# GreenleafLab/NucleoATAC

Measured on AMD Instinct MI355X. Metric: Mbp/s through occ+nuc signal pipeline, higher is better.
Workload: dtype f64

## Files before the change

nucleoatac_amd/csrc/natac_api.hip:

```cpp
#include "../../include/natac.h"
#ifndef NATAC_GNBL
#define NATAC_GNBL 2
#endif
#include "natac_kernels.hpp"
#include "natac_fft_bg.hpp"
#include "natac_occ_fast.hpp"
#include "natac_cand.hpp"
#include "natac_covsweep.hpp"
#include "natac_textz.hpp"
#include "natac_cores.hpp"
#include "natac_writer.hpp"
#include "natac_tabix.hpp"
#include "natac_pack.hpp"
#include "natac_bam.hpp"
#include "natac_bam_dev.hpp"
#include "natac_fasta.hpp"
#include "natac_fuzzfit.hpp"
#include "natac_bedtab.hpp"
#include "natac_pwmfit.hpp"
#include "natac_sites.hpp"
#include "natac_tracks.hpp"

#include <algorithm>
#include <cmath>
#include <cstdarg>
#include <cstdio>
#include <cstring>
#include <limits>
#include <string>
#include <vector>

using namespace natac;

static thread_local std::string g_err;

static int fail(int code, const char *fmt, ...) {
    char buf[512];
    va_list ap;
    va_start(ap, fmt);
    vsnprintf(buf, sizeof buf, fmt, ap);
    va_end(ap);
    g_err = buf;
    return code;
}

#define HIPCHK(expr)                                                                                  \
    do {                                                                                              \
        hipError_t e_ = (expr);                                                                       \
        if (e_ != hipSuccess)                                                                         \
            return fail(e_ == hipErrorOutOfMemory ? NATAC_E_NOMEM : NATAC_E_HIP, "%s: %s (%s:%d)", #expr, \
                        hipGetErrorString(e_), __FILE__, __LINE__);                                   \
    } while (0)

static hipError_t pool_alloc(void **p, size_t bytes);
static void dev_free(void *p);

template <class T>
class PoolBuf {
  public:
    PoolBuf() = default;
    PoolBuf(PoolBuf &&o) noexcept : p_(o.p_), n_(o.n_) { o.p_ = nullptr; o.n_ = 0; }
    PoolBuf &operator=(PoolBuf &&o) noexcept {
        if (this != &o) { reset(); p_ = o.p_; n_ = o.n_; o.p_ = nullptr; o.n_ = 0; }
        return *this;
    }
    ~PoolBuf() { reset(); }
    void reset() { dev_free(p_); p_ = nullptr; n_ = 0; }
    hipError_t alloc(size_t n) {
        reset();
        if (n == 0) n = 1;
        void *p = nullptr;
        const hipError_t e = pool_alloc(&p, n * sizeof(T));
        if (e == hipSuccess) { p_ = (T *)p; n_ = n; }
        return e;
    }
    T *get() const { return p_; }
    operator T *() const { return p_; }
    size_t size() const { return n_; }

  private:
    T *p_ = nullptr;
    size_t n_ = 0;
};

template <class T>
static int dev_alloc(PoolBuf<T> &buf, size_t n) {
    HIPCHK(buf.alloc(n));
    return NATAC_OK;
}

struct natac_ctx {
    int device = 0;
    hipStream_t stream = nullptr;
    hipStream_t copy_stream = nullptr;
    hipDeviceProp_t prop;
    PoolBuf<double> d_vmat, d_vmat_pad, d_srow, d_sizes;
    PoolBuf<double> d_lrt;
    long long lrt_gen = -1;
    int vlower = 0, vupper = 0, vw = 0, R = 0, W = 0, sizes_upper = 0;
    bool have_vmat = false, have_sizes = false, srow_dirty = true;
    bool vmat_zero = false, srow_zero = false;
    long long model_gen = 0;
    PoolBuf<double> d_fft_tw, d_fft_k;
    PoolBuf<double> d_fft_mtab, d_fft_swt;
    bool bg_ext = true;
    bool fft_dirty = true, bg_direct = false, occ_ordered = true, occ_zero_nfr = false;
    std::vector<double> h_sizes;
    PoolBuf<double> d_nucp, d_nfrp, d_alphas;
    int occ_upper = 0, n_alpha = 0, step = 0, halfstep = 0, flank = 0;
    double cutoff = 0;
    bool have_occ = false;
    int occ_zero_flags = 0;
    PoolBuf<double> d_occ_q4, d_occ_rho;
    int occ_nm = 0;
    bool occ_fast_ok = false, occ_force_general = false, occ_rn16 = false;
    double occ_b_floor = 0;
    PoolBuf<double> d_win_nuc, d_win_occ;
    PoolBuf<double> d_wb_occ;
    int wb_M = 0, wb_step = 0;
    int win_nuc_M = 0, win_occ_M = 0;
    double win_nuc_sd = -1, win_occ_sd = -1;
    double win_nuc_sum = 0, win_occ_sum = 0;
    bool profiling = false;
    struct Ev { int k; hipEvent_t a, b; hipStream_t st; };
    std::vector<Ev> pending;
    double prof_ms[NATAC_K_COUNT] = {0};
    int64_t prof_n[NATAC_K_COUNT] = {0};
    hipEvent_t t0 = nullptr, t1 = nullptr;
    hipStream_t ck_stream = nullptr;
    hipEvent_t ck_start = nullptr;
    long long *d_ck = nullptr;
    int ck_cap = 0;
    bool ck_active = false;
    struct Iv { int k; float t0, t1; };
    std::vector<Iv> ck_iv;
    PoolBuf<natac_text::P10> d_p10;
    PoolBuf<natac_deflate::CrcTables> d_crc;
};

struct natac_bam {
    natac_bamio::Bam *impl = nullptr;
};

enum TrackState : unsigned char { TS_EMPTY = 0, TS_PENDING, TS_RUN , TS_HOST  };
struct BatchOutputs {
    TrackState track[NATAC_T_COUNT] = {};
    bool grids = false;
    long long bg_gen = -1;
    int nuc_w = -1, nuc_upper = -1;
    bool occ_cov_by_nuc = false;
};

struct natac_batch {
    natac_ctx *ctx = nullptr;
    int nc = 0;
    long long nf = 0, nb = 0, total_bp = 0, total_grid = 0;
    int bias_left = 0, bias_right = 0;
    std::vector<int> h_len;
    std::vector<long long> h_out_off, h_grid_off;
    PoolBuf<int> d_len, d_lpos, d_ilen, d_centre, d_status;
    PoolBuf<long long> d_frag_off, d_bias_off, d_out_off, d_grid_off;
    PoolBuf<double> d_bias, d_ebias;
    PoolBuf<unsigned long long> d_occ_minkey;
    PoolBuf<int> d_occ_nan;
    int n_tiles_os = 0, os_width = 0;
    PoolBuf<int2> d_tiles_os, d_tiles1k;
    int n_tiles1k = 0;
    PoolBuf<int2> d_tiles256, d_tiles_bg, d_tiles_occ, d_ranges_occ, d_ranges256;
    PoolBuf<long long> d_tile256_first;
    PoolBuf<int> d_order_occ;
    int ranges256_w = -1;
    int ranges_occ_key[3] = {-1, -1, -1};
    int n_tiles256 = 0, n_tiles_bg = 0, n_tiles_occ = 0, bgG = 0;
    int grid_step = 0, grid_half = 0;
    PoolBuf<long long> d_blk_off;
    long long total_blocks = 0;
    PoolBuf<double> d_gsum;
    PoolBuf<int2> d_tiles_gs;
    int n_tiles_gs = 0, gs_Q = -1;
    PoolBuf<int> d_defer;
// ... 102 lines not shown
}

static hipError_t pool_mem_info(int dev, size_t *avail, size_t *total) {
    size_t fr = 0, tot = 0;
    hipError_t e = hipMemGetInfo(&fr, &tot);
    if (e != hipSuccess) return e;
    std::lock_guard<std::mutex> lk(g_pool.mu);
    for (auto &kv : g_pool.free_blocks[dev & 15]) fr += kv.first;
    *avail = fr;
    *total = tot;
    return hipSuccess;
}

static void dev_free(void *p) {
    if (!p) return;
    std::lock_guard<std::mutex> lk(g_pool.mu);
    auto it = g_pool.live.find(p);
    if (it == g_pool.live.end()) { (void)hipFree(p); return; }
    const int dev = it->second.first;
    const size_t bytes = it->second.second;
    g_pool.live.erase(it);
    if (g_pool.enabled) g_pool.free_blocks[dev].insert({bytes, p});
    else (void)hipFree(p);
}

template <class T>
static int dev_upload(natac_ctx *c, PoolBuf<T> &buf, const T *src, size_t n) {
    int rc = dev_alloc(buf, n);
    if (rc) return rc;
    if (n) HIPCHK(hipMemcpyAsync(buf, src, n * sizeof(T), hipMemcpyHostToDevice, c->stream));
    return NATAC_OK;
}

class StreamTemps {
  public:
    explicit StreamTemps(natac_ctx *c) : c_(c) {}
    ~StreamTemps() {
        if (!bufs_.empty() && hipStreamQuery(c_->stream) != hipSuccess) (void)hipStreamSynchronize(c_->stream);
    }
    template <class T>
    int alloc(T **p, size_t n) {
        bufs_.emplace_back();
        int rc = dev_alloc(bufs_.back(), std::max<size_t>(n, 1) * sizeof(T));
        *p = (T *)bufs_.back().get();
        return rc;
    }
    template <class T>
    int upload(T **p, const T *src, size_t n) {
        int rc = alloc(p, n);
        if (rc) return rc;
        if (n) HIPCHK(hipMemcpyAsync(*p, src, n * sizeof(T), hipMemcpyHostToDevice, c_->stream));
        return NATAC_OK;
    }

  private:
    natac_ctx *c_;
    std::vector<PoolBuf<unsigned char>> bufs_;
};

static int choose_bg_G(const natac_batch *b, int W) {
    const int cand[4] = {7, 9, 13, 17};
    double best = 1e300;
    int bestG = 9;
    const int stride = std::max(1, b->nc / 65536);
    for (int ci = 0; ci < 4; ++ci) {
        const int G = cand[ci], TW = 64 * G;
        double cost = 0;
        for (int i = 0; i < b->nc; i += stride) {
            const int nt = (b->h_len[i] + TW - 1) / TW;
            cost += (double)nt * (TW + (W - 1) * 0.15 * 8);
        }
        if (cost < best) { best = cost; bestG = G; }
    }
    return bestG;
}

static void launch_candidates(natac_ctx *c, const ChunkTable &ct, const VMatDev &vm, const int *d_cc, const int *d_cp, long long n,
                              const double *nuc_cov, const double *norm, const double *bnum, const double *bcov, double *lr,
                              double *var, double *z, const long long *tile_first = nullptr, const int2 *ranges256 = nullptr) {
    const int EW = c->W + ((c->vupper - 2) >> 1) + ((c->vupper - 1) >> 1);
    const int ZN = (((c->vupper - 2) >> 1) + ((c->vupper - 1) >> 1) + 5 + 32) & ~1, ON = (c->W + 1) & ~1;
    const size_t lds4 = ((size_t)4 * CAND_PER_WAVE * ((EW + 1) & ~1) + ZN + ON) * sizeof(double);
    const bool per_wave = c->W <= 2 * WAVE;
    const size_t ldsp = (size_t)4 * CAND_PER_WAVE * CANDP_STRIDE * sizeof(double);
    bool paired = per_wave && bnum && bcov && c->vlower >= 2 && (c->R & 1) == 0 && c->W >= 64 && !vm.has_zero && EW <= CANDP_STRIDE &&
                  !getenv("NATAC_CAND_FULL") && !getenv("NATAC_CAND_OLD");
    if (paired && (c->lrt_gen != c->model_gen || !c->d_lrt)) {
        if (c->d_lrt.size() < (size_t)c->R * c->W && dev_alloc(c->d_lrt, (size_t)c->R * c->W) != NATAC_OK)
            paired = false;
        if (paired) {
            hipLaunchKernelGGL(natac_lr_table, dim3((unsigned)((c->R * c->W + 255) / 256)), dim3(256), 0, c->stream, c->d_vmat, c->d_srow, c->R, c->W,
                               c->d_lrt);
            c->lrt_gen = c->model_gen;
        }
    }
    if (paired) {
        VMatDev vml = vm;
        vml.lrt = c->d_lrt;
        const long long per_block = 4 * CAND_PER_WAVE;
        const dim3 grid((unsigned)((n + per_block - 1) / per_block));
        if (c->vlower & 1)
            hipLaunchKernelGGL((natac_candidates_paired<true>), grid, dim3(256), ldsp, c->stream, ct, vml, d_cc, d_cp, (int)n, nuc_cov, norm,
                               bnum, bcov, tile_first, ranges256, lr, var, z);
        else
            hipLaunchKernelGGL((natac_candidates_paired<false>), grid, dim3(256), ldsp, c->stream, ct, vml, d_cc, d_cp, (int)n, nuc_cov, norm,
                               bnum, bcov, tile_first, ranges256, lr, var, z);
        return;
    }
    if (per_wave && lds4 <= 64 * 1024) {
        const long long per_block = 4 * CAND_PER_WAVE;
        if (bnum && bcov && !getenv("NATAC_CAND_FULL"))
            hipLaunchKernelGGL((natac_candidates4<true>), dim3((unsigned)((n + per_block - 1) / per_block)), dim3(256), lds4, c->stream,
                               ct, vm, d_cc, d_cp, (int)n, nuc_cov, norm, bnum, bcov, lr, var, z);
        else
            hipLaunchKernelGGL((natac_candidates4<false>), dim3((unsigned)((n + per_block - 1) / per_block)), dim3(256), lds4, c->stream,
                               ct, vm, d_cc, d_cp, (int)n, nuc_cov, norm, bnum, bcov, lr, var, z);
    } else {
        hipLaunchKernelGGL(natac_candidates, dim3((unsigned)n), dim3(256), (size_t)(EW + 2) * sizeof(double), c->stream, ct, vm, d_cc,
                           d_cp, nuc_cov, norm, lr, var, z);
    }
}

template <int G>
static void launch_bg(natac_batch *b, const ChunkTable &ct, const VMatDev &vm) {
    natac_ctx *c = b->ctx;
    constexpr int W = 121;
    const int PW = 64 * G + W - 1;
    const int EW = PW + ((vm.upper - 2) >> 1) + ((vm.upper - 1) >> 1);
    const size_t lds = ((size_t)((EW + 1) & ~1) + PW) * sizeof(double);
    hipLaunchKernelGGL((natac_background<G, W>), dim3(b->n_tiles_bg), dim3(64), lds, c->stream, ct, b->d_tiles_bg, vm,
                       b->d_track[NATAC_T_NUC_COV], b->d_track[NATAC_T_RAW], b->d_track[NATAC_T_BACKGROUND],
                       b->d_track[NATAC_T_NORM], b->d_bnum, b->d_bcov);
}


static int ensure_text_tables(natac_ctx *c) {
    if (c->d_p10 && c->d_crc) return NATAC_OK;
    int rc;
    if (!c->d_p10 && (rc = dev_upload(c, c->d_p10, natac_text::H_P10, sizeof(natac_text::H_P10) / sizeof(natac_text::P10)))) return rc;
    if (!c->d_crc) {
        natac_deflate::CrcTables t;
        natac_deflate::crc_init(t);
        if ((rc = dev_upload(c, c->d_crc, &t, 1))) return rc;
    }
    HIPCHK(hipStreamSynchronize(c->stream));
    return NATAC_OK;
}

template <class T>
static int dev_scan(natac_ctx *c, const T *in, long long n, unsigned long long *out, StreamTemps &tmp) {
    using namespace natac_textz;
    const long long nblk = (n + SCAN_PER_BLOCK - 1) / SCAN_PER_BLOCK;
    unsigned long long *sums = nullptr;
    int rc = tmp.alloc(&sums, (size_t)nblk + 1);
    if (rc) return rc;
    hipLaunchKernelGGL((tz_scan_block_sums<T>), dim3((unsigned)nblk), dim3(256), 0, c->stream, in, n, sums);
    hipLaunchKernelGGL(tz_scan_sums, dim3(1), dim3(1024), 0, c->stream, sums, nblk);
    hipLaunchKernelGGL((tz_scan_final<T>), dim3((unsigned)nblk), dim3(256), 0, c->stream, in, n, sums, out);
    hipError_t e = hipGetLastError();
    if (e != hipSuccess) return fail(NATAC_E_HIP, "scan: %s", hipGetErrorString(e));
    return NATAC_OK;
}

static int dev_scan2(natac_ctx *c, const unsigned char *in, long long n, unsigned long long *out_sum, unsigned long long *out_cnt, StreamTemps &tmp) {
    using namespace natac_textz;
    const long long nblk = (n + SCAN_PER_BLOCK - 1) / SCAN_PER_BLOCK;
    unsigned long long *sums = nullptr;
    int rc = tmp.alloc(&sums, 2 * ((size_t)nblk + 1));
    if (rc) return rc;
    hipLaunchKernelGGL(tz_scan2_block_sums, dim3((unsigned)nblk), dim3(256), 0, c->stream, in, n, nblk, sums);
    hipLaunchKernelGGL(tz_scan_sums, dim3(1), dim3(1024), 0, c->stream, sums, nblk);
    hipLaunchKernelGGL(tz_scan_sums, dim3(1), dim3(1024), 0, c->stream, sums + nblk + 1, nblk);
    hipLaunchKernelGGL(tz_scan2_final, dim3((unsigned)nblk), dim3(256), 0, c->stream, in, n, nblk, sums, out_sum, out_cnt);
    hipError_t e = hipGetLastError();
    if (e != hipSuccess) return fail(NATAC_E_HIP, "scan: %s", hipGetErrorString(e));
    return NATAC_OK;
}

static int format_values(natac_batch *b, const double *d_vals, const int32_t *chrom_id, const char *const *names, int32_t n_names,
                         const int64_t *chunk_start, int write_zero, int compress, int64_t *n_bytes, int64_t *n_text_bytes, int64_t *n_lines,
                         int32_t *n_hard) {
    using namespace natac_textz;
    natac_ctx *c = b->ctx;
    int rc = ensure_text_tables(c);
    if (rc) return rc;
    b->d_fmt_out.reset();
    b->fmt_bytes = -1;
    b->fmt_groups.clear();
// ... 471 lines not shown
    int rc = dev_upload(b->ctx, b->d_tiles_bg, tiles.data(), tiles.size());
    if (rc) return rc;
    HIPCHK(sync_all(b->ctx));
    return NATAC_OK;
}

static int ensure_fft(natac_ctx *c) {
    int rc;
    if (!c->d_fft_tw) {
        std::vector<double> tw(2 * (size_t)natac::FFT_N);
        for (int k = 0; k < natac::FFT_N; ++k) {
            const double a = 2.0 * M_PI * k / natac::FFT_N;
            tw[2 * k] = std::cos(a);
            tw[2 * k + 1] = -std::sin(a);
        }
        if (const char *e = getenv("NATAC_FAULT_TWIDDLE")) {
            int k = 0; double dlt = 0.0;
            if (sscanf(e, "%d:%lf", &k, &dlt) == 2 && k >= 0 && k < natac::FFT_N) tw[2 * (size_t)k] += dlt;
        }
        if ((rc = dev_upload(c, c->d_fft_tw, tw.data(), tw.size()))) return rc;
        HIPCHK(sync_all(c));
    }
    if (!c->fft_dirty) return NATAC_OK;
    HIPCHK(sync_all(c));
    const int npair = (c->R + 1) / 2;
    if ((rc = dev_alloc(c->d_fft_k, (size_t)npair * 2 * natac::FFT_N))) return rc;
    hipLaunchKernelGGL(natac_fft_template, dim3(npair), dim3(64), 0, c->stream, c->d_vmat, c->d_srow, c->R, c->W, c->d_fft_tw, c->d_fft_k);
    if (c->W >= natac::FFT_EXT) {
        c->d_fft_mtab.reset(); c->d_fft_swt.reset();
        const int NJ = (c->R + 3) / 4;
        if ((rc = dev_alloc(c->d_fft_mtab, (size_t)2 * NJ * 64)) || (rc = dev_alloc(c->d_fft_swt, (size_t)4 * NJ))) return rc;
        hipLaunchKernelGGL(natac_fft_edge_table_mfma, dim3((2 * NJ * 64 + 255) / 256), dim3(256), 0, c->stream, c->d_vmat, c->d_srow, c->R, c->W, NJ,
                           c->d_fft_mtab, c->d_fft_swt);
    }
    HIPCHK(hipGetLastError());
    c->fft_dirty = false;
    return NATAC_OK;
}

static int ensure_window(natac_ctx *c, PoolBuf<double> &slot, int *slotM, double *slotsd, int M, double sd, double *slotsum = nullptr) {
    if (slot && *slotM == M && *slotsd == sd) return NATAC_OK;
    HIPCHK(sync_all(c));
    std::vector<double> w((size_t)M);
    for (int i = 0; i < M; ++i) {
        double n = (double)i - (M - 1) / 2.0;
        double q = n / sd;
        w[i] = std::exp(-0.5 * (q * q));
    }
    int rc = dev_upload(c, slot, w.data(), (size_t)M);
    if (rc) return rc;
    HIPCHK(sync_all(c));
    if (slotsum) {
        double acc = 0.0;
        for (int i = 0; i < M; ++i) acc = acc + w[i];
        *slotsum = acc;
    }
    *slotM = M;
    *slotsd = sd;
    return NATAC_OK;
}

static int run_exp_bias(natac_batch *b, hipStream_t st, bool from_occ) {
    if (!b->d_bias) return NATAC_OK;
    if (from_occ && b->ebias_fresh) { b->ebias_fresh = false; return NATAC_OK; }
    b->ebias_fresh = !from_occ;
    int rc;
    if (!b->d_ebias && (rc = dev_alloc(b->d_ebias, (size_t)b->nb))) return rc;
    const int blocks = (int)std::min<long long>((b->nb + 255) / 256, 16384);
    hipLaunchKernelGGL(natac_exp_bias, dim3(blocks), dim3(256), 0, st, b->d_bias, b->d_ebias, b->nb);
    return NATAC_OK;
}

static ChunkTable make_table(natac_batch *b) {
    ChunkTable t;
    t.nc = b->nc; t.chunk_len = b->d_len; t.frag_off = b->d_frag_off; t.lpos = b->d_lpos; t.ilen = b->d_ilen;
    t.centre = b->d_centre; t.bias_off = b->d_bias_off; t.bias = b->d_bias; t.ebias = b->d_ebias; t.bias_left = b->bias_left;
    t.bias_right = b->bias_right; t.out_off = b->d_out_off; t.grid_off = b->d_grid_off;
    return t;
}
static VMatDev make_vmat(natac_ctx *c) {
    VMatDev v;
    v.mat = c->d_vmat; v.matp = c->d_vmat_pad; v.srow = c->d_srow; v.lower = c->vlower; v.upper = c->vupper; v.w = c->vw; v.R = c->R; v.W = c->W;
    v.has_zero = (c->vmat_zero || c->srow_zero) ? 1 : 0;
    v.lrt = nullptr;
    return v;
}
static OccModelDev make_occ(natac_ctx *c) {
    OccModelDev o;
    o.nuc_probs = c->d_nucp; o.nfr_probs = c->d_nfrp; o.alphas = c->d_alphas; o.upper = c->occ_upper;
    o.n_alpha = c->n_alpha; o.step = c->step; o.halfstep = c->halfstep; o.flank = c->flank; o.cutoff = c->cutoff;
    o.ci_factor = std::exp(-0.5 * c->cutoff);
    o.zero_flags = c->occ_zero_flags;
    o.b_floor = c->occ_b_floor;
    return o;
}

static int build_tiles(natac_batch *b, int width, PoolBuf<int2> &d_out, int *n_out, bool grid_units = false, int step = 1, int half = 0) {
    std::vector<int2> tiles;
    tiles.reserve((size_t)(b->total_bp / std::max(1, width)) + b->nc);
    for (int i = 0; i < b->nc; ++i) {
        int n = b->h_len[i];
        if (grid_units) n = (b->h_len[i] > half) ? (b->h_len[i] - half + step - 1) / step : 0;
        for (int x = 0; x < n; x += width) tiles.push_back(make_int2(i, x));
    }
    *n_out = (int)tiles.size();
    int rc = dev_upload(b->ctx, d_out, tiles.data(), tiles.size());
    if (rc) return rc;
    HIPCHK(sync_all(b->ctx));
    return NATAC_OK;
}

int natac_batch_create(natac_ctx *c, int32_t nc, const int32_t *chunk_len, const int64_t *frag_off, const int32_t *frag_lpos,
                       const int32_t *frag_ilen, const int64_t *bias_off, const double *bias_log, int32_t bias_left,
                       int32_t bias_right, natac_batch **out) {
    if (!c || !out || !chunk_len || !frag_off) return fail(NATAC_E_ARG, "null argument");
    *out = nullptr;
    if (nc <= 0) return fail(NATAC_E_ARG, "n_chunks must be positive");
    if (bias_log && !bias_off) return fail(NATAC_E_ARG, "bias_log without bias_off");
    if (frag_off[0] != 0) return fail(NATAC_E_ARG, "frag_off[0] must be 0");
    const long long nf = frag_off[nc];
    if (nf > 0 && (!frag_lpos || !frag_ilen)) return fail(NATAC_E_ARG, "fragment arrays are NULL");
    HIPCHK(hipSetDevice(c->device));
    natac_batch *b = new natac_batch();
    b->ctx = c; b->nc = nc; b->nf = nf; b->bias_left = bias_left; b->bias_right = bias_right;
    b->h_len.assign(chunk_len, chunk_len + nc);
    b->h_out_off.resize((size_t)nc + 1);
    b->h_out_off[0] = 0;
    for (int i = 0; i < nc; ++i) {
        if (chunk_len[i] <= 0) { delete b; return fail(NATAC_E_ARG, "chunk %d has length %d", i, chunk_len[i]); }
        if (frag_off[i + 1] < frag_off[i] || frag_off[i + 1] - frag_off[i] > 0x7fffffffLL) {
            delete b; return fail(NATAC_E_ARG, "frag_off not monotone (chunk %d)", i);
        }
        if (bias_off && bias_off[i + 1] - bias_off[i] != (long long)chunk_len[i] + bias_left + bias_right) {
            delete b; return fail(NATAC_E_ARG, "bias slice of chunk %d must cover [start-%d, end+%d)", i, bias_left, bias_right);
        }
        b->h_out_off[i + 1] = b->h_out_off[i] + chunk_len[i];
    }
    b->total_bp = b->h_out_off[nc];
    b->nb = bias_off ? bias_off[nc] : 0;
    auto upload = [&]() -> int {
        int rc;
        if ((rc = dev_upload(c, b->d_len, chunk_len, (size_t)nc)) ||
            (rc = dev_upload(c, b->d_frag_off, (const long long *)frag_off, (size_t)nc + 1)) ||
            (rc = dev_upload(c, b->d_lpos, frag_lpos, (size_t)nf)) || (rc = dev_upload(c, b->d_ilen, frag_ilen, (size_t)nf)) ||
            (rc = dev_alloc(b->d_centre, (size_t)nf)) || (rc = dev_upload(c, b->d_out_off, b->h_out_off.data(), (size_t)nc + 1)))
            return rc;
        if (bias_off) {
            if ((rc = dev_upload(c, b->d_bias_off, (const long long *)bias_off, (size_t)nc + 1))) return rc;
            if (bias_log) rc = dev_upload(c, b->d_bias, bias_log, (size_t)b->nb);
            else rc = dev_alloc(b->d_bias, (size_t)b->nb);
            if (rc) return rc;
        }
        if ((rc = dev_alloc(b->d_status, (size_t)nc))) return rc;
        hipError_t e = hipMemsetAsync(b->d_status, 0, (size_t)nc * sizeof(int), c->stream);
        if (e != hipSuccess) return fail(NATAC_E_HIP, "memset: %s", hipGetErrorString(e));
        if (nf > 0) {
            int blocks = (int)std::min<long long>((nf + 255) / 256, 4096);
            hipLaunchKernelGGL(natac_frag_centres, dim3(blocks), dim3(256), 0, c->stream, b->d_lpos, b->d_ilen, b->d_centre, nf);
        }
        if ((rc = build_tiles(b, 256, b->d_tiles256, &b->n_tiles256))) return rc;
        {
            std::vector<long long> first((size_t)nc + 1, 0);
            for (int i = 0; i < nc; ++i) first[(size_t)i + 1] = first[i] + (chunk_len[i] + 255) / 256;
            if ((rc = dev_upload(c, b->d_tile256_first, first.data(), first.size()))) return rc;
        }
        e = hipStreamSynchronize(c->stream);
        if (e != hipSuccess) return fail(NATAC_E_HIP, "upload: %s", hipGetErrorString(e));
// ... 2392 lines not shown
```

nucleoatac_amd/csrc/natac_cand.hpp:

```cpp
#pragma once
#include "natac_kernels.hpp"

namespace natac {

__device__ __forceinline__ int row_lower_bound(const int *__restrict__ a, int lo, int hi, int key, int l, int sh) {
    while (__ballot(hi - lo > 16) != 0ull) {
        const int n = hi - lo;
        const bool big = n > 16;
        const int stride = big ? (n + 15) / 16 : 1;
        const int pi = min((l + 1) * stride - 1, max(n - 1, 0));
        const bool less = big && a[lo + pi] < key;
        const int cnt = __popc((unsigned)(__ballot(less) >> sh) & 0xffffu);
        if (big) {
            lo = min(lo + cnt * stride, hi);
            hi = min(lo + stride, hi);
        }
    }
    const int i = lo + l;
    const bool less = (i < hi) && a[i] < key;
    return lo + __popc((unsigned)(__ballot(less) >> sh) & 0xffffu);
}

__global__ void __launch_bounds__(256) natac_lr_table(const double *__restrict__ vmat, const double *__restrict__ srow, int R, int W,
                                                        double *__restrict__ out) {
    const int i = blockIdx.x * 256 + threadIdx.x;
    if (i < R * W) out[i] = log(vmat[i] / srow[i / W]);
}

constexpr int CANDP_STRIDE = 376;

template <bool LODD>
__global__ void __launch_bounds__(256) __attribute__((amdgpu_waves_per_eu(3, 3))) natac_candidates_paired(
    ChunkTable ct, VMatDev vm, const int *__restrict__ cand_chunk, const int *__restrict__ cand_pos, int ncand,
    const double *__restrict__ nuc_cov, const double *__restrict__ norm, const double *__restrict__ bnum,
    const double *__restrict__ bcov, const long long *__restrict__ tile_first, const int2 *__restrict__ ranges256,
    double *__restrict__ out_lr, double *__restrict__ out_var, double *__restrict__ out_z) {
    extern __shared__ __attribute__((aligned(16))) double smem[];
    constexpr int Q = CAND_PER_WAVE;
    const int A = (vm.upper - 2) >> 1, Bh = (vm.upper - 1) >> 1;
    const int W = vm.W, R = vm.R;
    const int EW = W + A + Bh;
    constexpr int EWP = CANDP_STRIDE;
    const int wave = threadIdx.x >> 6, lane = threadIdx.x & 63;
    double *Ew = smem + wave * Q * EWP;
    const int k0 = (blockIdx.x * 4 + wave) * Q;
    if (k0 >= ncand) return;
    int chunk[Q], pos[Q];
    bool esmall = false;
#pragma unroll
    for (int q = 0; q < Q; ++q) {
        const int k = (k0 + q < ncand) ? k0 + q : k0;
        chunk[q] = cand_chunk[k];
        pos[q] = cand_pos[k];
        const int L = ct.chunk_len[chunk[q]];
        const double *b = ct.bias ? ct.ebias + ct.bias_off[chunk[q]] : nullptr;
        const int nb = L + ct.bias_left + ct.bias_right;
        const int j0 = pos[q] - vm.w - A + ct.bias_left;
        double emin = __builtin_inf();
        for (int u = lane; u < EW; u += WAVE) {
            const int j = j0 + u;
            double e = 1.0;
            if (b) e = (j >= 0 && j < nb) ? b[j] : 0.0;
            Ew[q * EWP + u] = e;
            emin = fmin(emin, e);
        }
        esmall |= !(wave_min(emin) > 0x1p-500);
    }
    __builtin_amdgcn_wave_barrier();
    const int c1 = lane, c2 = min(lane + WAVE, W - 1);
    const bool h2 = lane + WAVE < W;
    double a1[Q][2], a2[Q][2];
    double carry[Q][2];
#pragma unroll
    for (int q = 0; q < Q; ++q) { a1[q][0] = a1[q][1] = a2[q][0] = a2[q][1] = 0.0; }
    const int m0 = LODD ? (vm.lower - 1) >> 1 : vm.lower >> 1;
    {
        const int off = LODD ? A + m0 : A - m0 + 1;
#pragma unroll
        for (int q = 0; q < Q; ++q) { carry[q][0] = Ew[q * EWP + c1 + off]; carry[q][1] = Ew[q * EWP + c2 + off]; }
    }
    const double *__restrict__ vmat = vm.mat;
    const int npair = R >> 1;
    const double *psh1 = Ew + c1 + (LODD ? A - m0 : A + m0), *psh2 = Ew + c2 + (LODD ? A - m0 : A + m0);
    const double *pnw1 = Ew + c1 + (LODD ? A + m0 + 1 : A - m0), *pnw2 = Ew + c2 + (LODD ? A + m0 + 1 : A - m0);
    constexpr int DSH = LODD ? -1 : 1, DNW = LODD ? 1 : -1;
    struct PairT { double va0, va1, vb0, vb1, sa, sb; };
    const double hm = h2 ? 1.0 : 0.0;
    const unsigned o1 = (unsigned)c1 * 8u, o2 = (unsigned)c2 * 8u;
    auto load_pair = [&](int k) {
        PairT t;
        t.sa = vm.srow[2 * k]; t.sb = vm.srow[2 * k + 1];
        const char *ra = (const char *)(vmat + (size_t)(2 * k) * (size_t)W), *rb = ra + (size_t)W * sizeof(double);
        t.va0 = *(const double *)(ra + o1); t.va1 = *(const double *)(ra + o2);
        t.vb0 = *(const double *)(rb + o1); t.vb1 = *(const double *)(rb + o2);
        return t;
    };
    auto pair_step = [&](const PairT &t, const double (&cin)[Q][2], double (&cout)[Q][2]) {
        const double va0 = t.va0, va1 = hm * t.va1, vb0 = t.vb0, vb1 = hm * t.vb1;
        const double wa0 = t.sa * (va0 * va0), wa1 = t.sa * (va1 * va1);
        const double wb0 = t.sb * (vb0 * vb0), wb1 = t.sb * (vb1 * vb1);
        double s0[Q], s1[Q];
#pragma unroll
        for (int q = 0; q < Q; ++q) {
            s0[q] = psh1[q * EWP]; s1[q] = psh2[q * EWP];
            cout[q][0] = pnw1[q * EWP]; cout[q][1] = pnw2[q * EWP];
        }
        __builtin_amdgcn_sched_barrier(0);
#pragma unroll
        for (int q = 0; q < Q; ++q) {
            const double n0 = cout[q][0], n1 = cout[q][1];
            a1[q][0] = fma(s0[q], fma(vb0, n0, va0 * cin[q][0]), a1[q][0]);
            a1[q][1] = fma(s1[q], fma(vb1, n1, va1 * cin[q][1]), a1[q][1]);
            a2[q][0] = fma(s0[q], fma(wb0, n0, wa0 * cin[q][0]), a2[q][0]);
            a2[q][1] = fma(s1[q], fma(wb1, n1, wa1 * cin[q][1]), a2[q][1]);
        }
        psh1 += DSH; psh2 += DSH; pnw1 += DNW; pnw2 += DNW;
    };
    double carry2[Q][2];
    int k = 0;
    PairT t0 = load_pair(0), t1 = load_pair(min(1, npair - 1));
    for (; k + 4 <= npair; k += 4) {
        const PairT u0 = load_pair(min(k + 2, npair - 1));
        pair_step(t0, carry, carry2);
        const PairT u1 = load_pair(min(k + 3, npair - 1));
        pair_step(t1, carry2, carry);
        t0 = load_pair(min(k + 4, npair - 1));
        pair_step(u0, carry, carry2);
        t1 = load_pair(min(k + 5, npair - 1));
        pair_step(u1, carry2, carry);
    }
    for (; k + 2 <= npair; k += 2) {
        const PairT u0 = load_pair(min(k + 2, npair - 1));
        pair_step(t0, carry, carry2);
        t0 = u0;
        const PairT u1 = load_pair(min(k + 3, npair - 1));
        pair_step(t1, carry2, carry);
        t1 = u1;
    }
    if (k < npair) pair_step(t0, carry, carry2);
    bool zero[Q];
#pragma unroll
    for (int q = 0; q < Q; ++q) zero[q] = false;
    if (esmall) {
        for (int r = 0; r < R; ++r) {
            const int i = vm.lower + r;
            const int hl = floor_half(i - 1), hr = floor_half(i);
            const double sr = vm.srow[r];
            const double v1 = vmat[r * W + c1], v2 = vmat[r * W + c2];
#pragma unroll
            for (int q = 0; q < Q; ++q) {
                const double *e = Ew + q * EWP;
                const double b1 = e[c1 + A - hl] * e[c1 + A + hr], b2 = e[c2 + A - hl] * e[c2 + A + hr];
                zero[q] |= (v1 * b1 == 0.0 || sr * b1 == 0.0) || (h2 && (v2 * b2 == 0.0 || sr * b2 == 0.0));
            }
        }
    }
    double tBV2[Q], tB0V[Q];
    bool anyzero[Q];
#pragma unroll
    for (int q = 0; q < Q; ++q) {
        tB0V[q] = wave_sum(a1[q][0] + a1[q][1]);
        tBV2[q] = wave_sum(a2[q][0] + a2[q][1]);
        anyzero[q] = __ballot(zero[q]) != 0ull;
    }
    const int row = lane >> 4, l = lane & 15, sh = 16 * row;
    int mych = chunk[0], myp = pos[0];
    double myB0V = tB0V[0], myBV2 = tBV2[0];
    bool myzero = anyzero[0];
#pragma unroll
    for (int q = 1; q < Q; ++q)
        if (row == q) { mych = chunk[q]; myp = pos[q]; myB0V = tB0V[q]; myBV2 = tBV2[q]; myzero = anyzero[q]; }
    const long long op = ct.out_off[mych] + myp;
    const double tB = bcov[op], tBV = bnum[op];
    const int nfr = (int)(ct.frag_off[mych + 1] - ct.frag_off[mych]);
    const int *cen = ct.centre + ct.frag_off[mych];
    const int *iln = ct.ilen + ct.frag_off[mych];
    int f0, f1;
    if (ranges256) {
        const int2 tr = ranges256[tile_first[mych] + (myp >> 8)];
        const int klo = myp - vm.w, khi = myp + vm.w + 1;
        int below_lo = 0, below_hi = 0;
        int span = tr.y - tr.x;
        span = max(max(__builtin_amdgcn_readlane(span, 0), __builtin_amdgcn_readlane(span, 16)),
                   max(__builtin_amdgcn_readlane(span, 32), __builtin_amdgcn_readlane(span, 48)));
        for (int base = 0; base < span; base += 64) {
            int cv[4];
#pragma unroll
            for (int it = 0; it < 4; ++it) {
                const int i = tr.x + base + 16 * it + l;
                cv[it] = 0x7fffffff;
                if (i < tr.y) cv[it] = cen[i];
            }
#pragma unroll
            for (int it = 0; it < 4; ++it) {
                below_lo += __popc((unsigned)(__ballot(cv[it] < klo) >> sh) & 0xffffu);
                below_hi += __popc((unsigned)(__ballot(cv[it] < khi) >> sh) & 0xffffu);
            }
        }
        f0 = tr.x + below_lo;
        f1 = tr.x + below_hi;
    } else {
        f0 = row_lower_bound(cen, 0, nfr, myp - vm.w, l, sh);
        f1 = row_lower_bound(cen, f0, nfr, myp + vm.w + 1, l, sh);
    }
    const double *__restrict__ lrt = vm.lrt;
    double acc = 0.0, cntf = 0.0;
    int fmax = f1 - f0;
    fmax = max(max(__builtin_amdgcn_readlane(fmax, 0), __builtin_amdgcn_readlane(fmax, 16)),
               max(__builtin_amdgcn_readlane(fmax, 32), __builtin_amdgcn_readlane(fmax, 48)));
    {
        int nn[4], cc[4];
#pragma unroll
        for (int it = 0; it < 4; ++it) {
            const int f = f0 + 16 * it + l;
            nn[it] = -1; cc[it] = 0;
            if (f < f1) { nn[it] = iln[f]; cc[it] = cen[f]; }
        }
        double tv[4];
#pragma unroll
        for (int it = 0; it < 4; ++it) {
            tv[it] = 0.0;
            if (nn[it] >= vm.lower && nn[it] < vm.upper) tv[it] = lrt[(nn[it] - vm.lower) * W + (cc[it] - myp + vm.w)];
        }
#pragma unroll
        for (int it = 0; it < 4; ++it)
            if (nn[it] >= vm.lower && nn[it] < vm.upper) { acc += tv[it]; cntf += 1.0; }
    }
    for (int base = 64; base < fmax; base += 16) {
        const int f = f0 + base + l;
        if (f < f1) {
            const int n = iln[f];
            if (n >= vm.lower && n < vm.upper) { acc += lrt[(n - vm.lower) * W + (cen[f] - myp + vm.w)]; cntf += 1.0; }
        }
    }
    acc = row_sum(acc);
    cntf = row_sum(cntf);
    const double nl = acc, ul = cntf * log(myB0V / tB);
    if (l == 0 && k0 + row < ncand) {
        const double m1 = tBV / tB;
        const int reads = (int)nuc_cov[op];
        const double var = (double)reads * (myBV2 / tB - m1 * m1);
        out_lr[k0 + row] = myzero ? __builtin_nan("") : (nl - ul);
        out_var[k0 + row] = var;
        out_z[k0 + row] = norm[op] / sqrt(var);
    }
// ... 4 lines not shown
```

nucleoatac_amd/csrc/natac_kernels.hpp:

```cpp
#pragma once
#include <hip/hip_runtime.h>
#include <stdint.h>

#include <type_traits>

namespace natac {

constexpr int WAVE = 64;

struct ChunkTable {
    int nc;
    const int *chunk_len;
    const long long *frag_off;
    const int *lpos;
    const int *ilen;
    const int *centre;
    const long long *bias_off;
    const double *bias;
    const double *ebias;
    int bias_left, bias_right;
    const long long *out_off;
    const long long *grid_off;
};

constexpr int VPAD = 128;

struct VMatDev {
    const double *mat;
    const double *matp;
    const double *srow;
    const double *lrt;
    int lower, upper, w, R, W;
    int has_zero;
};

__device__ __forceinline__ int floor_half(int x) { return x >> 1; }

__device__ __forceinline__ int lower_bound_i32(const int *a, int lo, int hi, int key) {
    while (lo < hi) {
        int mid = (lo + hi) >> 1;
        if (a[mid] < key) lo = mid + 1; else hi = mid;
    }
    return lo;
}

template <int CTRL>
__device__ __forceinline__ double dpp_mov_f64(double v) {
    const int lo = __builtin_amdgcn_update_dpp(0, __double2loint(v), CTRL, 0xf, 0xf, false);
    const int hi = __builtin_amdgcn_update_dpp(0, __double2hiint(v), CTRL, 0xf, 0xf, false);
    return __hiloint2double(hi, lo);
}
__device__ __forceinline__ double readlane_f64(double v, int lane) {
    const int lo = __builtin_amdgcn_readlane(__double2loint(v), lane);
    const int hi = __builtin_amdgcn_readlane(__double2hiint(v), lane);
    return __hiloint2double(hi, lo);
}
__device__ __forceinline__ double wave_sum(double v) {
    v += dpp_mov_f64<0xB1>(v);
    v += dpp_mov_f64<0x4E>(v);
    v += dpp_mov_f64<0x141>(v);
    v += dpp_mov_f64<0x140>(v);
    return (readlane_f64(v, 0) + readlane_f64(v, 16)) + (readlane_f64(v, 32) + readlane_f64(v, 48));
}
__device__ __forceinline__ double wave_min(double v) {
    v = fmin(v, dpp_mov_f64<0xB1>(v));
    v = fmin(v, dpp_mov_f64<0x4E>(v));
    v = fmin(v, dpp_mov_f64<0x141>(v));
    v = fmin(v, dpp_mov_f64<0x140>(v));
    return fmin(fmin(readlane_f64(v, 0), readlane_f64(v, 16)), fmin(readlane_f64(v, 32), readlane_f64(v, 48)));
}
__device__ __forceinline__ double wave_max(double v) {
    v = fmax(v, dpp_mov_f64<0xB1>(v));
    v = fmax(v, dpp_mov_f64<0x4E>(v));
    v = fmax(v, dpp_mov_f64<0x141>(v));
    v = fmax(v, dpp_mov_f64<0x140>(v));
    return fmax(fmax(readlane_f64(v, 0), readlane_f64(v, 16)), fmax(readlane_f64(v, 32), readlane_f64(v, 48)));
}
__device__ __forceinline__ int wave_or(int v) {
    int r = 0;
#pragma unroll
    for (int bit = 1; bit <= 8; bit <<= 1)
        if (__ballot((v & bit) != 0) != 0ull) r |= bit;
    return r;
}
__device__ __forceinline__ double row_sum(double v) {
    v += dpp_mov_f64<0xB1>(v);
    v += dpp_mov_f64<0x4E>(v);
    v += dpp_mov_f64<0x141>(v);
    v += dpp_mov_f64<0x140>(v);
    return v;
}
__device__ __forceinline__ double row_max(double v) {
    v = fmax(v, dpp_mov_f64<0xB1>(v));
    v = fmax(v, dpp_mov_f64<0x4E>(v));
    v = fmax(v, dpp_mov_f64<0x141>(v));
    v = fmax(v, dpp_mov_f64<0x140>(v));
    return v;
}
template <int CTRL>
__device__ __forceinline__ int dpp_mov_i32(int v) { return __builtin_amdgcn_update_dpp(0, v, CTRL, 0xf, 0xf, false); }
__device__ __forceinline__ int row_min_i32(int v) {
    v = min(v, dpp_mov_i32<0xB1>(v));
    v = min(v, dpp_mov_i32<0x4E>(v));
    v = min(v, dpp_mov_i32<0x141>(v));
    v = min(v, dpp_mov_i32<0x140>(v));
    return v;
}
__device__ __forceinline__ int row_max_i32(int v) {
    v = max(v, dpp_mov_i32<0xB1>(v));
    v = max(v, dpp_mov_i32<0x4E>(v));
    v = max(v, dpp_mov_i32<0x141>(v));
    v = max(v, dpp_mov_i32<0x140>(v));
    return v;
}
// ... 2115 lines not shown
```

Before: 3489.

## Remap paired candidate kernel to adjacent-column lanes with split even/odd LDS planes

In the paired candidate kernel each lane now owns two adjacent columns (2l, 2l+1) instead of columns l and l+64. The V matrix is copied into a zero-padded 128-column buffer so each lane loads a row pair with one double2 load. The bias window in LDS is stored as separate even and odd planes so the shifted diagonal reads become contiguous, and the reads are rotated through registers so each step needs fewer LDS loads. This adds a padded matrix buffer, a larger LDS footprint and more complex indexing, which risks mistakes at odd W or at the tail loop.

```diff
diff --git a/nucleoatac_amd/csrc/natac_api.hip b/nucleoatac_amd/csrc/natac_api.hip
--- a/nucleoatac_amd/csrc/natac_api.hip
+++ b/nucleoatac_amd/csrc/natac_api.hip
@@ -95,7 +95,7 @@
     hipStream_t copy_stream = nullptr;
     hipDeviceProp_t prop;
     PoolBuf<double> d_vmat, d_vmat_pad, d_srow, d_sizes;
-    PoolBuf<double> d_lrt;
+    PoolBuf<double> d_lrt, d_matc;
     long long lrt_gen = -1;
     int vlower = 0, vupper = 0, vw = 0, R = 0, W = 0, sizes_upper = 0;
     bool have_vmat = false, have_sizes = false, srow_dirty = true;
@@ -364,28 +364,30 @@
     const int ZN = (((c->vupper - 2) >> 1) + ((c->vupper - 1) >> 1) + 5 + 32) & ~1, ON = (c->W + 1) & ~1;
     const size_t lds4 = ((size_t)4 * CAND_PER_WAVE * ((EW + 1) & ~1) + ZN + ON) * sizeof(double);
     const bool per_wave = c->W <= 2 * WAVE;
-    const size_t ldsp = (size_t)4 * CAND_PER_WAVE * CANDP_STRIDE * sizeof(double);
     bool paired = per_wave && bnum && bcov && c->vlower >= 2 && (c->R & 1) == 0 && c->W >= 64 && !vm.has_zero && EW <= CANDP_STRIDE &&
                   !getenv("NATAC_CAND_FULL") && !getenv("NATAC_CAND_OLD");
-    if (paired && (c->lrt_gen != c->model_gen || !c->d_lrt)) {
-        if (c->d_lrt.size() < (size_t)c->R * c->W && dev_alloc(c->d_lrt, (size_t)c->R * c->W) != NATAC_OK)
+    if (paired && (c->lrt_gen != c->model_gen || !c->d_lrt || !c->d_matc)) {
+        const size_t ncell = (size_t)c->R * CANDP_COLS;
+        if ((c->d_lrt.size() < (size_t)c->R * c->W && dev_alloc(c->d_lrt, (size_t)c->R * c->W) != NATAC_OK) ||
+            (c->d_matc.size() < ncell && dev_alloc(c->d_matc, ncell) != NATAC_OK))
             paired = false;
         if (paired) {
-            hipLaunchKernelGGL(natac_lr_table, dim3((unsigned)((c->R * c->W + 255) / 256)), dim3(256), 0, c->stream, c->d_vmat, c->d_srow, c->R, c->W,
-                               c->d_lrt);
+            hipLaunchKernelGGL(natac_lr_table, dim3((unsigned)((ncell + 255) / 256)), dim3(256), 0, c->stream, c->d_vmat, c->d_srow, c->R, c->W,
+                               c->d_lrt, c->d_matc);
             c->lrt_gen = c->model_gen;
         }
     }
     if (paired) {
         VMatDev vml = vm;
         vml.lrt = c->d_lrt;
+        vml.matc = c->d_matc;
         const long long per_block = 4 * CAND_PER_WAVE;
         const dim3 grid((unsigned)((n + per_block - 1) / per_block));
         if (c->vlower & 1)
-            hipLaunchKernelGGL((natac_candidates_paired<true>), grid, dim3(256), ldsp, c->stream, ct, vml, d_cc, d_cp, (int)n, nuc_cov, norm,
+            hipLaunchKernelGGL((natac_candidates_paired<true>), grid, dim3(256), CANDP_LDS, c->stream, ct, vml, d_cc, d_cp, (int)n, nuc_cov, norm,
                                bnum, bcov, tile_first, ranges256, lr, var, z);
         else
-            hipLaunchKernelGGL((natac_candidates_paired<false>), grid, dim3(256), ldsp, c->stream, ct, vml, d_cc, d_cp, (int)n, nuc_cov, norm,
+            hipLaunchKernelGGL((natac_candidates_paired<false>), grid, dim3(256), CANDP_LDS, c->stream, ct, vml, d_cc, d_cp, (int)n, nuc_cov, norm,
                                bnum, bcov, tile_first, ranges256, lr, var, z);
         return;
     }
@@ -1023,7 +1025,7 @@
     VMatDev v;
     v.mat = c->d_vmat; v.matp = c->d_vmat_pad; v.srow = c->d_srow; v.lower = c->vlower; v.upper = c->vupper; v.w = c->vw; v.R = c->R; v.W = c->W;
     v.has_zero = (c->vmat_zero || c->srow_zero) ? 1 : 0;
-    v.lrt = nullptr;
+    v.lrt = nullptr; v.matc = nullptr;
     return v;
 }
 static OccModelDev make_occ(natac_ctx *c) {
diff --git a/nucleoatac_amd/csrc/natac_cand.hpp b/nucleoatac_amd/csrc/natac_cand.hpp
--- a/nucleoatac_amd/csrc/natac_cand.hpp
+++ b/nucleoatac_amd/csrc/natac_cand.hpp
@@ -21,13 +21,23 @@
     return lo + __popc((unsigned)(__ballot(less) >> sh) & 0xffffu);
 }
 
+constexpr int CANDP_STRIDE = 376;
+constexpr int CANDP_PLANE = CANDP_STRIDE / 2 + 1;
+constexpr size_t CANDP_LDS = (size_t)4 * CAND_PER_WAVE * 2 * CANDP_PLANE * sizeof(double);
+constexpr int CANDP_COLS = 128;
+
 __global__ void __launch_bounds__(256) natac_lr_table(const double *__restrict__ vmat, const double *__restrict__ srow, int R, int W,
-                                                        double *__restrict__ out) {
+                                                        double *__restrict__ out, double *__restrict__ matc) {
     const int i = blockIdx.x * 256 + threadIdx.x;
-    if (i < R * W) out[i] = log(vmat[i] / srow[i / W]);
-}
-
-constexpr int CANDP_STRIDE = 376;
+    const int r = i / CANDP_COLS, c = i % CANDP_COLS;
+    if (r >= R) return;
+    double v = 0.0;
+    if (c < W) {
+        v = vmat[r * W + c];
+        out[r * W + c] = log(v / srow[r]);
+    }
+    matc[i] = v;
+}
 
 template <bool LODD>
 __global__ void __launch_bounds__(256) __attribute__((amdgpu_waves_per_eu(3, 3))) natac_candidates_paired(
@@ -40,7 +50,7 @@
     const int A = (vm.upper - 2) >> 1, Bh = (vm.upper - 1) >> 1;
     const int W = vm.W, R = vm.R;
     const int EW = W + A + Bh;
-    constexpr int EWP = CANDP_STRIDE;
+    constexpr int EPL = CANDP_PLANE, EWP = 2 * EPL;
     const int wave = threadIdx.x >> 6, lane = threadIdx.x & 63;
     double *Ew = smem + wave * Q * EWP;
     const int k0 = (blockIdx.x * 4 + wave) * Q;
@@ -57,91 +67,105 @@
         const int nb = L + ct.bias_left + ct.bias_right;
         const int j0 = pos[q] - vm.w - A + ct.bias_left;
         double emin = __builtin_inf();
-        for (int u = lane; u < EW; u += WAVE) {
+        for (int u = lane; u <= EW; u += WAVE) {
             const int j = j0 + u;
-            double e = 1.0;
-            if (b) e = (j >= 0 && j < nb) ? b[j] : 0.0;
-            Ew[q * EWP + u] = e;
-            emin = fmin(emin, e);
+            double e = 0.0;
+            if (u < EW) {
+                e = 1.0;
+                if (b) e = (j >= 0 && j < nb) ? b[j] : 0.0;
+                emin = fmin(emin, e);
+            }
+            Ew[q * EWP + (u & 1) * EPL + (u >> 1)] = e;
         }
         esmall |= !(wave_min(emin) > 0x1p-500);
     }
     __builtin_amdgcn_wave_barrier();
-    const int c1 = lane, c2 = min(lane + WAVE, W - 1);
-    const bool h2 = lane + WAVE < W;
-    double a1[Q][2], a2[Q][2];
-    double carry[Q][2];
-#pragma unroll
-    for (int q = 0; q < Q; ++q) { a1[q][0] = a1[q][1] = a2[q][0] = a2[q][1] = 0.0; }
+    const int ll = min(lane, (W - 1) >> 1);
+    const int first = 2 * ll + 1 < W ? 1 : 0;
+    double ax[Q][2], ay[Q][2];
+#pragma unroll
+    for (int q = 0; q < Q; ++q) { ax[q][0] = ax[q][1] = ay[q][0] = ay[q][1] = 0.0; }
     const int m0 = LODD ? (vm.lower - 1) >> 1 : vm.lower >> 1;
-    {
-        const int off = LODD ? A + m0 : A - m0 + 1;
-#pragma unroll
-        for (int q = 0; q < Q; ++q) { carry[q][0] = Ew[q * EWP + c1 + off]; carry[q][1] = Ew[q * EWP + c2 + off]; }
-    }
-    const double *__restrict__ vmat = vm.mat;
+    auto elem = [&](int o) { return Ew + (o & 1) * EPL + ll + (o >> 1); };
+    const int os0 = LODD ? A - m0 : A + m0 + 1;
+    const int on1 = LODD ? A + m0 + 2 : A - m0;
+    constexpr int DS = LODD ? -1 : 1, DN = LODD ? 1 : -1;
+    double sA[Q], sB[Q], nA[Q], nB[Q], nC[Q], nD[Q];
+#pragma unroll
+    for (int q = 0; q < Q; ++q) {
+        sB[q] = elem(os0 - (LODD ? first : 1) * DS)[q * EWP];
+        nA[q] = elem(on1 - (LODD ? 2 : 1 + first) * DN)[q * EWP];
+        nB[q] = elem(on1 - DN)[q * EWP];
+    }
+    const double *ps0 = elem(os0), *ps1 = elem(os0 + DS), *pn0 = elem(on1), *pn1 = elem(on1 + DN);
     const int npair = R >> 1;
-    const double *psh1 = Ew + c1 + (LODD ? A - m0 : A + m0), *psh2 = Ew + c2 + (LODD ? A - m0 : A + m0);
-    const double *pnw1 = Ew + c1 + (LODD ? A + m0 + 1 : A - m0), *pnw2 = Ew + c2 + (LODD ? A + m0 + 1 : A - m0);
-    constexpr int DSH = LODD ? -1 : 1, DNW = LODD ? 1 : -1;
-    struct PairT { double va0, va1, vb0, vb1, sa, sb; };
-    const double hm = h2 ? 1.0 : 0.0;
-    const unsigned o1 = (unsigned)c1 * 8u, o2 = (unsigned)c2 * 8u;
+    struct PairT { double2 va, vb; double sa, sb; };
+    const double2 *__restrict__ vrow = (const double2 *)vm.matc + lane;
     auto load_pair = [&](int k) {
         PairT t;
         t.sa = vm.srow[2 * k]; t.sb = vm.srow[2 * k + 1];
-        const char *ra = (const char *)(vmat + (size_t)(2 * k) * (size_t)W), *rb = ra + (size_t)W * sizeof(double);
-        t.va0 = *(const double *)(ra + o1); t.va1 = *(const double *)(ra + o2);
-        t.vb0 = *(const double *)(rb + o1); t.vb1 = *(const double *)(rb + o2);
+        t.va = vrow[(size_t)(2 * k) * (CANDP_COLS / 2)];
+        t.vb = vrow[(size_t)(2 * k + 1) * (CANDP_COLS / 2)];
         return t;
     };
-    auto pair_step = [&](const PairT &t, const double (&cin)[Q][2], double (&cout)[Q][2]) {
-        const double va0 = t.va0, va1 = hm * t.va1, vb0 = t.vb0, vb1 = hm * t.vb1;
-        const double wa0 = t.sa * (va0 * va0), wa1 = t.sa * (va1 * va1);
-        const double wb0 = t.sb * (vb0 * vb0), wb1 = t.sb * (vb1 * vb1);
-        double s0[Q], s1[Q];
+    auto pair_step = [&](auto Jc, const PairT &t, const double (&sp)[Q], double (&sc)[Q], const double (&np)[Q],
+                         const double (&nc)[Q], double (&nn)[Q]) {
+        constexpr int J = decltype(Jc)::value;
+        const double vax = LODD ? t.va.x : t.va.y, vay = LODD ? t.va.y : t.va.x;
+        const double vbx = LODD ? t.vb.x : t.vb.y, vby = LODD ? t.vb.y : t.vb.x;
+        const double wax = t.sa * (vax * vax), way = t.sa * (vay * vay);
+        const double wbx = t.sb * (vbx * vbx), wby = t.sb * (vby * vby);
+        const double *ps = (J & 1) ? ps1 : ps0, *pn = (J & 1) ? pn1 : pn0;
 #pragma unroll
         for (int q = 0; q < Q; ++q) {
-            s0[q] = psh1[q * EWP]; s1[q] = psh2[q * EWP];
-            cout[q][0] = pnw1[q * EWP]; cout[q][1] = pnw2[q * EWP];
+            sc[q] = ps[q * EWP + (J >> 1) * DS];
+            nn[q] = pn[q * EWP + (J >> 1) * DN];
         }
         __builtin_amdgcn_sched_barrier(0);
 #pragma unroll
         for (int q = 0; q < Q; ++q) {
-            const double n0 = cout[q][0], n1 = cout[q][1];
-            a1[q][0] = fma(s0[q], fma(vb0, n0, va0 * cin[q][0]), a1[q][0]);
-            a1[q][1] = fma(s1[q], fma(vb1, n1, va1 * cin[q][1]), a1[q][1]);
-            a2[q][0] = fma(s0[q], fma(wb0, n0, wa0 * cin[q][0]), a2[q][0]);
-            a2[q][1] = fma(s1[q], fma(wb1, n1, wa1 * cin[q][1]), a2[q][1]);
-        }
-        psh1 += DSH; psh2 += DSH; pnw1 += DNW; pnw2 += DNW;
+            ax[q][0] = fma(sc[q], fma(vbx, nc[q], vax * np[q]), ax[q][0]);
+            ay[q][0] = fma(sp[q], fma(vby, nn[q], vay * nc[q]), ay[q][0]);
+            ax[q][1] = fma(sc[q], fma(wbx, nc[q], wax * np[q]), ax[q][1]);
+            ay[q][1] = fma(sp[q], fma(wby, nn[q], way * nc[q]), ay[q][1]);
+        }
     };
-    double carry2[Q][2];
+    auto advance = [&](int pairs) {
+        ps0 += (pairs >> 1) * DS; ps1 += (pairs >> 1) * DS; pn0 += (pairs >> 1) * DN; pn1 += (pairs >> 1) * DN;
+    };
+    using J0 = std::integral_constant<int, 0>; using J1 = std::integral_constant<int, 1>;
+    using J2 = std::integral_constant<int, 2>; using J3 = std::integral_constant<int, 3>;
     int k = 0;
     PairT t0 = load_pair(0), t1 = load_pair(min(1, npair - 1));
     for (; k + 4 <= npair; k += 4) {
         const PairT u0 = load_pair(min(k + 2, npair - 1));
-        pair_step(t0, carry, carry2);
+        pair_step(J0(), t0, sB, sA, nA, nB, nC);
         const PairT u1 = load_pair(min(k + 3, npair - 1));
-        pair_step(t1, carry2, carry);
+        pair_step(J1(), t1, sA, sB, nB, nC, nD);
         t0 = load_pair(min(k + 4, npair - 1));
-        pair_step(u0, carry, carry2);
+        pair_step(J2(), u0, sB, sA, nC, nD, nA);
         t1 = load_pair(min(k + 5, npair - 1));
-        pair_step(u1, carry2, carry);
-    }
-    for (; k + 2 <= npair; k += 2) {
+        pair_step(J3(), u1, sA, sB, nD, nA, nB);
+        advance(4);
+    }
+    if (k + 2 <= npair) {
         const PairT u0 = load_pair(min(k + 2, npair - 1));
-        pair_step(t0, carry, carry2);
+        pair_step(J0(), t0, sB, sA, nA, nB, nC);
+        pair_step(J1(), t1, sA, sB, nB, nC, nD);
+        advance(2);
         t0 = u0;
-        const PairT u1 = load_pair(min(k + 3, npair - 1));
-        pair_step(t1, carry2, carry);
-        t1 = u1;
-    }
-    if (k < npair) pair_step(t0, carry, carry2);
+#pragma unroll
+        for (int q = 0; q < Q; ++q) { nA[q] = nC[q]; nB[q] = nD[q]; }
+        k += 2;
+    }
+    if (k < npair) pair_step(J0(), t0, sB, sA, nA, nB, nC);
     bool zero[Q];
 #pragma unroll
     for (int q = 0; q < Q; ++q) zero[q] = false;
     if (esmall) {
+        const double *__restrict__ vmat = vm.mat;
+        const int c1 = min(2 * lane, W - 1), c2 = min(2 * lane + 1, W - 1);
+        const bool h1 = 2 * lane < W, h2 = 2 * lane + 1 < W;
         for (int r = 0; r < R; ++r) {
             const int i = vm.lower + r;
             const int hl = floor_half(i - 1), hr = floor_half(i);
@@ -150,8 +174,9 @@
 #pragma unroll
             for (int q = 0; q < Q; ++q) {
                 const double *e = Ew + q * EWP;
-                const double b1 = e[c1 + A - hl] * e[c1 + A + hr], b2 = e[c2 + A - hl] * e[c2 + A + hr];
-                zero[q] |= (v1 * b1 == 0.0 || sr * b1 == 0.0) || (h2 && (v2 * b2 == 0.0 || sr * b2 == 0.0));
+                auto E = [&](int u) { return e[(u & 1) * EPL + (u >> 1)]; };
+                const double b1 = E(c1 + A - hl) * E(c1 + A + hr), b2 = E(c2 + A - hl) * E(c2 + A + hr);
+                zero[q] |= (h1 && (v1 * b1 == 0.0 || sr * b1 == 0.0)) || (h2 && (v2 * b2 == 0.0 || sr * b2 == 0.0));
             }
         }
     }
@@ -159,8 +184,8 @@
     bool anyzero[Q];
 #pragma unroll
     for (int q = 0; q < Q; ++q) {
-        tB0V[q] = wave_sum(a1[q][0] + a1[q][1]);
-        tBV2[q] = wave_sum(a2[q][0] + a2[q][1]);
+        tB0V[q] = wave_sum(ax[q][0] + ay[q][0]);
+        tBV2[q] = wave_sum(ax[q][1] + ay[q][1]);
         anyzero[q] = __ballot(zero[q]) != 0ull;
     }
     const int row = lane >> 4, l = lane & 15, sh = 16 * row;
diff --git a/nucleoatac_amd/csrc/natac_kernels.hpp b/nucleoatac_amd/csrc/natac_kernels.hpp
--- a/nucleoatac_amd/csrc/natac_kernels.hpp
+++ b/nucleoatac_amd/csrc/natac_kernels.hpp
@@ -30,6 +30,7 @@
     const double *matp;
     const double *srow;
     const double *lrt;
+    const double *matc;
     int lower, upper, w, R, W;
     int has_zero;
 };
```

Measured after the change: 3549 (median of 6 runs). +1.7%, better.
